# amathislab/BUCTD

Hardware: AMD Instinct MI355X
Metric: images/sec (train) BUCTD-CoAM-W48 384x288 (higher is better)
Workload: dtype f32 (3x3 convs: operands split exactly into 3 bf16 pieces, 6 bf16 MFMAs per product, fp32 accumulate - fp32-class); 1 GPU; BUCTD-CoAM-W48 (pose_hrnet_coam, ATT_MODULES [F,T,F,F], colored condition) 384x288 CrowdPose-14kpt full train step: fwd + JointsMSE + bwd + grad all-reduce + Adam + arg-max accuracy decode; global_batch=32, batch_per_gpu=32, input=N x 6 x 384 x 288 fp32, params=115581770, parallelism=dp1, hip_streams=4, conv_math=bf16x6, step_graph=False

## Files before the change

### buctd_amd/_C.py

```python
import ctypes as C
import os

import torch

_HERE = os.path.dirname(os.path.abspath(__file__))
LIB_PATH = os.path.join(_HERE, "lib", "libbuctd_hip.so")


class ConvDesc(C.Structure):
    _fields_ = [(n, C.c_int) for n in ("N", "H", "W", "Ci", "Co", "R", "S", "stride", "pad", "Ho", "Wo")]


class BasicBlockDesc(C.Structure):
    _fields_ = ([(n, C.c_int) for n in ("N", "H", "W", "C")] +
                [(n, C.c_void_p) for n in ("x", "w1_fwd", "w2_fwd", "w1_bwd", "w2_bwd", "gamma1", "beta1", "gamma2", "beta2",
                                           "running_mean1", "running_var1", "running_mean2", "running_var2")] +
                [(n, C.c_float) for n in ("eps1", "momentum1", "eps2", "momentum2")] +
                [(n, C.c_void_p) for n in ("z1", "z2", "y", "acc", "stat")])


class BasicBlockGrads(C.Structure):
    _fields_ = ([(n, C.c_void_p) for n in ("dy", "dz2", "dres", "dy1", "dz1", "dx", "dw1", "dw2", "dgamma1", "dbeta1",
                                           "dgamma2", "dbeta2")] +
                [(n, C.c_int) for n in ("acc_w1", "acc_w2", "acc_bn1", "acc_bn2")] +
# ... 9 lines not shown
class C3Conv(C.Structure):
    _fields_ = ([(n, C.c_int) for n in ("N", "H", "W", "Ci", "Co")] +
                [(n, C.c_void_p) for n in ("x", "wprep", "residual")] + [("relu", C.c_int)] +
                [(n, C.c_void_p) for n in ("y", "stats_acc")] + [("in_bn", C.POINTER(BnAccIn))] +
                [(n, C.c_void_p) for n in ("in_gamma", "in_beta")] + [("in_relu", C.c_int)] +
                [(n, C.c_void_p) for n in ("bn_z", "bn_y", "bn_mean", "bn_invstd", "bn_gamma", "bn_beta", "bn_acc")])


class C3ConvEval(C.Structure):
    _fields_ = ([(n, C.c_int) for n in ("N", "H", "W", "Ci", "Co")] +
                [(n, C.c_void_p) for n in ("x", "wprep", "scale", "shift", "residual")] + [("relu", C.c_int), ("y", C.c_void_p)])


class BnApplyItem(C.Structure):
    _fields_ = [("z", C.c_void_p), ("st", BnAccIn), ("gamma", C.c_void_p), ("beta", C.c_void_p), ("residual", C.c_void_p),
                ("relu", C.c_int), ("y", C.c_void_p), ("rows", C.c_long), ("C", C.c_int)]


class BnBwdItem(C.Structure):
    _fields_ = ([(n, C.c_void_p) for n in ("dy", "y", "z", "mean", "invstd", "gamma", "beta")] +
                [("relu", C.c_int), ("rows", C.c_long), ("C", C.c_int)] +
                [(n, C.c_void_p) for n in ("dz", "dres", "dgamma", "dbeta")] +
                [("accumulate", C.c_int), ("acc", C.c_void_p), ("acc_ready", C.c_int)])


class Wg3Conv(C.Structure):
    _fields_ = ([(n, C.c_int) for n in ("N", "H", "W", "Ci", "Co")] +
                [(n, C.c_void_p) for n in ("x", "dy", "dw")] + [("accumulate", C.c_int)] +
                [(n, C.c_void_p) for n in ("x_mean", "x_invstd", "x_gamma", "x_beta")] + [("x_relu", C.c_int)] +
                [("workspace", C.c_void_p), ("workspace_bytes", C.c_size_t)])


class MhaArgs(C.Structure):
    _fields_ = ([(n, C.c_int) for n in ("B", "T", "h", "dh")] +
                [(n, C.c_void_p) for n in ("q", "k", "v")] + [(n, C.c_int) for n in ("ldq", "ldk", "ldv")] +
                [("out", C.c_void_p), ("ldo", C.c_int), ("lse", C.c_void_p), ("scale", C.c_float), ("p_drop", C.c_float),
                 ("dout", C.c_void_p), ("lddo", C.c_int)] +
                [(n, C.c_void_p) for n in ("dq", "dk", "dv")] + [(n, C.c_int) for n in ("lddq", "lddk", "lddv")])


class RefineArgs(C.Structure):
    _fields_ = ([(n, C.c_void_p) for n in ("coords", "maxvals", "offset", "center", "scale", "box_score", "items",
                                           "cond_trunc", "cond_joints", "status", "hist_preds", "hist_score",
                                           "hist_box_score", "hist_keypoint_score", "hist_center", "hist_scale")] +
                [(n, C.c_int) for n in ("B", "K", "pass_", "passes", "heatmap_w", "heatmap_h", "crop_w", "crop_h")] +
                [(n, C.c_double) for n in ("margin", "aspect_ratio", "in_vis_thre", "scale_thre")])
# ... 135 lines not shown
    "buctd_joints_ohkm_mse_workspace": (_SZ, [_I, _I]),
    "buctd_joints_ohkm_mse": (_I, [_P, _P, _P, _I, _I, _I, _I, _P, _P, _F, _P, _SZ, _P]),
    "buctd_argmax_decode": (_I, [_P, _I, _I, _I, _P, _P, _P, _P]),
    "buctd_warp_affine_norm": (_I, [_P, _I, _I, _I, _P, _P, _P, _L, _P, _P]),
    "buctd_cond_render_into": (_I, [_P, _I, _P, _I, _I, _I, _I, _I, _I, _P, _L, _P, _SZ, _P]),
    "buctd_cond_geometry": (_I, [_P, _P, _P, _P, _I, _I, _P, _P, _P, _P]),
    "buctd_cond_mirror": (_I, [_P, _I, _P, _P, _I, _I, _I, _P, _P]),
    "buctd_mirror_rows": (_I, [_P, _L, _P, _L, _P, _I, _I, _I, _I, _I, _P]),
    "buctd_refine_step": (_I, [C.POINTER(RefineArgs), _P]),
    "buctd_sample_geometry": (_I, [C.POINTER(SampleGeomArgs), _P]),
    "buctd_synthesize_pose": (_I, [_P, _P, _P, _P, _P, _P, _I, _I, _I, C.c_ulonglong, _P, _P]),
    "buctd_mha_fwd_supported": (_I, [_I, _I]),
    "buctd_mha_fwd": (_I, [_I, _I, _I, _P, _P, _P, _I, _I, _F, _P, _P, _P]),
    "buctd_mha_fwd_bf16x6": (_I, [_I, _I, _I, _P, _P, _P, _I, _I, _F, _P, _P, _P]),
    "buctd_gconv_x6_supported": (_I, [_I] * 7),
    "buctd_gconv_x6_prep_bytes": (_SZ, [_I, _I, _I, _I]),
    "buctd_gconv_x6_prep": (_I, [_I, _I, _I, _P, _I, _P, _P]),
    "buctd_gconv_x6_prep_item_bytes": (_SZ, []),
    "buctd_gconv_x6_prep_item": (_I, [_I, _I, _I, _P, _I, _P, _P]),
    "buctd_gconv_x6_prep_batched": (_I, [_P, _I, _P]),
    "buctd_gconv_x6_stats_groups": (_I, [_I] * 6 + [_PI, _PI]),
    "buctd_gconv_x6_fwd": (_I, [_I] * 6 + [_P] * 6 + [_I, _P, _P, _P, _P]),
    "buctd_gconv_x6_dgrad": (_I, [_I] * 6 + [_P] * 4 + [_P]),
    "buctd_mha_fwd_bf16x6_workspace": (_SZ, [_I, _I, _I]),
    "buctd_mha_fwd_bf16x6_ws": (_I, [_I, _I, _I, _P, _P, _P, _I, _I, _F, _P, _P, _P, _SZ, _P]),
    "buctd_mha_train_supported": (_I, [_I, _I]),
    "buctd_mha_fwd_train": (_I, [_I, _I, _I, _P, _P, _P, _I, _I, _F, _F, _U64, _P, _P, _P]),
    "buctd_mha_bwd_workspace": (_SZ, [_I, _I]),
    "buctd_mha_bwd": (_I, [_I, _I, _I, _P, _P, _P, _I, _I, _P, _P, _P, _F, _F, _U64, _P, _P, _I, _P, _I, _P, _SZ, _P]),
    "buctd_mha_fwd_train_dseed": (_I, [_I, _I, _I, _P, _P, _P, _I, _I, _F, _F, _P, _P, _P, _P]),
    "buctd_mha_bwd_dseed": (_I, [_I, _I, _I, _P, _P, _P, _I, _I, _P, _P, _P, _F, _F, _P, _P, _P, _I, _P, _I, _P, _SZ, _P]),
    "buctd_mha_heads_fwd_supported": (_I, [_I, _I, _I]),
    "buctd_mha_heads_fwd": (_I, [C.POINTER(MhaArgs), _P]),
    "buctd_mha_heads_fwd_bf16x6": (_I, [C.POINTER(MhaArgs), _P]),
    "buctd_mha_heads_train_supported": (_I, [_I, _I, _I]),
    "buctd_mha_heads_fwd_train": (_I, [C.POINTER(MhaArgs), _U64, _P]),
    "buctd_mha_heads_bwd_workspace": (_SZ, [_I, _I, _I]),
    "buctd_mha_heads_bwd": (_I, [C.POINTER(MhaArgs), _U64, _P, _SZ, _P]),
    "buctd_mha_heads_fwd_train_dseed": (_I, [C.POINTER(MhaArgs), _P, _P]),
    "buctd_mha_heads_bwd_dseed": (_I, [C.POINTER(MhaArgs), _P, _P, _SZ, _P]),
    "buctd_nms_workspace": (_SZ, [_I]),
    "buctd_nms": (_I, [_P, _P, _P, _I, _I, _F, _P, _SZ, _P]),
    "buctd_cpu_nms": (_I, [_P, _I, _P, _F, _P, _P]),
    "buctd_argmax_decode_refined": (_I, [_P, _I, _I, _I, _P, _P, _P, _P, _P]),
    "buctd_argmax_decode_dark": (_I, [_P, _I, _I, _I, _P, _P, _P, _P, _P]),
    "buctd_gaussian_target": (_I, [_P, _P, _I, _I, _I, _I, _F, _F, _F, _P, _P, _P]),
# ... 61 lines not shown
```

### buctd_amd/csrc/conv_gather_x6.hip

```cpp
#include "c3_lean.h"
#include <string.h>

#define GC_MAXT 9
#define GC_TAB_OFF (56 * 1024)

struct GcClass {
  int ntaps, nhs, nsteps;
  int oy0, ox0;
  long wp_off;
  unsigned pdy, pdx;
};

struct GcArgs {
  C3Args e;
  const float* src;
  const unsigned char* wp;
  int SH, SWd, SC, ss, cpt;
  int ncls;
  GcClass cls[4];
};

template <int MF, int NF, int WM, int WN, int MODE>
__global__ __launch_bounds__(256, 2) void gconv_x6_kernel(GcArgs p) {
  constexpr int BM = WM * MF * 16, BN = WN * NF * 16, ROWB = 96, PST = 32, BROW = 192;
  constexpr int QA = BM / 64;
  static_assert(WM * WN == 4 && BM % 64 == 0, "four waves, BM a multiple of 64");
  extern __shared__ __attribute__((aligned(16))) unsigned char smem[];
  const int t = threadIdx.x, lane = t & 63, wave = t >> 6;
  const int i16 = lane & 15, g = lane >> 4;
  const int wave_m = wave % WM, wave_n = wave / WM;
  const int bx = blockIdx.x, by = blockIdx.y;
  const GcClass& c = p.cls[blockIdx.z];
  C3Args e = p.e;
  e.oy0 = c.oy0; e.ox0 = c.ox0;
  const int p0 = bx * BM, n0 = by * BN;

  constexpr bool PRIV = WN == 1;
  constexpr int RSTEP = PRIV ? 16 : 64;
  static_assert(!PRIV || MF * 16 / 16 == QA, "wave-private staging: MF passes of 16 rows == BM / 64");
  unsigned rowbase[QA];
  unsigned tapok[QA];
  const int arow = PRIV ? wave * (MF * 16) + (lane >> 2) : (t >> 2), c4 = t & 3;
  const __amdgpu_buffer_rsrc_t r_src = c3_rsrc(p.src, (unsigned)e.N * p.SH * p.SWd * p.SC * 4u);
#pragma unroll
  for (int q = 0; q < QA; ++q) {
    const int pp = p0 + arow + RSTEP * q;
    const int n = fast_div(pp, e.ib_mul, e.ib_sh);
    const int rem = pp - n * e.IB;
    const int yy = fast_div(rem, e.sw_mul, e.sw_sh), xx = rem - yy * e.SW;
    const bool real = (pp < e.P) & (n < e.N) & (yy >= 1) & (xx >= 1) & (xx <= e.W);
    const int sy0 = (yy - 1) * p.ss, sx0 = (xx - 1) * p.ss;
    rowbase[q] = (unsigned)(((n * p.SH + sy0) * p.SWd + sx0) * p.SC + c4 * 4) * 4u;
    unsigned ok = 0u;
    for (int tp = 0; tp < c.ntaps; ++tp) {
      const int sy = sy0 + (int)((c.pdy >> (2 * tp)) & 3u) - 1, sx = sx0 + (int)((c.pdx >> (2 * tp)) & 3u) - 1;
// ... 84 lines not shown
    if (2 * QA > MF) {
#pragma unroll
      for (int i = MF; i < 2 * QA; ++i) {
        const int h = i / QA, q = i % QA;
        split_store_pk<3, PST>(smem + (size_t)(1 - SET) * ABUF + ((size_t)h * BM + arow + RSTEP * q) * ROWB, c4 * 4,
                               areg[1 - SET][h][q]);
      }
    }
    if (!PRIV) __syncthreads();
  };

  load_a(0, areg[0]);
  load_b(0, bnx[0]);
  load_a(1, areg[1]);
  store_a(areg[0], 0);
  if (!PRIV) __syncthreads();
  for (int st = 0; st < c.nsteps; st += 2) {
    step(st, IC<0>{});
    if (st + 1 < c.nsteps) step(st + 1, IC<1>{});
  }
  __syncthreads();
  if constexpr (MODE < 0) c3_epilogue<MF, NF, WM, WN>(e, acc, smem, bx, by, p0, n0);
  else c3l_epilogue<MF, NF, WM, WN, MODE>(e, acc, smem, reinterpret_cast<float*>(smem + GC_TAB_OFF), p0, n0);
}

struct GcPrep {
  const float* w;
  unsigned char* out;
  int Co, Ci, R, S, dir;
  int ncls;
  int ntaps[4], nsteps[4];
  long off[4];
  int tr[4][GC_MAXT], ts[4][GC_MAXT];
  long items[4];
};

__device__ __forceinline__ void gc_prep_body(const GcPrep& p) {
  const int nrows = p.dir ? p.Ci : p.Co, kc = p.dir ? p.Co : p.Ci, cpt = kc / 16;
  const long total = p.items[p.ncls - 1];
  for (long idx = (long)blockIdx.x * 256 + threadIdx.x; idx < total; idx += (long)gridDim.x * 256) {
    int cl = 0;
    while (idx >= p.items[cl]) ++cl;
    const long li = idx - (cl ? p.items[cl - 1] : 0);
    const int ks = (int)(li & 31);
    const long sr = li >> 5;
    const int row = (int)(sr % nrows), st = (int)(sr / nrows);
// ... 329 lines not shown
static bool r1_ok(int kind, long rows, int cin, int cout) {
  if (kind != 1 || cin % 32 || (cout != 64 && cout != 128 && cout != 256)) return false;
  const size_t lds = (size_t)(cin / 32) * cout * R1_WROW + (size_t)8 * R1_STG;
  return lds <= 150 * 1024 && (size_t)8 * cout * 16 <= (size_t)(cin / 32) * cout * R1_WROW && rows >= 65536;
}

static int r1_run(long rows, int cin, int cout, const float* x, const void* wprep, const float* bias, const float* residual, float* out,
                  long long* stats_acc, hipStream_t st, const char* who) {
  R1Args a;
  a.x = x; a.wp = (const unsigned char*)wprep; a.bias = bias; a.res = residual; a.out = out; a.stats_acc = stats_acc;
  a.rows = rows; a.Ci = cin; a.Co = cout; a.nblocks = (int)((rows + 31) / 32);
  const size_t lds = (size_t)(cin / 32) * cout * R1_WROW + (size_t)8 * R1_STG;
  static unsigned char done[3][BUCTD_MAX_DEVICES] = {{0}};
  void (*fn)(R1Args) = cout == 64 ? conv1x1_rows_x6_kernel<4> : cout == 128 ? conv1x1_rows_x6_kernel<8> : conv1x1_rows_x6_kernel<16>;
  if (const int rc = buctd_raise_lds_limit(reinterpret_cast<const void*>(fn), 160 * 1024, done[cout == 64 ? 0 : cout == 128 ? 1 : 2], who))
    return rc;
  int grid = 256;
  if (grid * 8 > a.nblocks) grid = (a.nblocks + 7) / 8;
  hipLaunchKernelGGL(fn, dim3(grid), dim3(512), lds, st, a);
  BUCTD_CHECK_LAUNCH(who);
  return BUCTD_OK;
}

static int gc_run(int kind, int dir, int N, int H, int W, int Ci, int Co, const float* src, const void* wprep, const float* bias,
                  const float* scale, const float* shift, const float* residual, int relu, float* out, float* stats_partials,
                  int* stats_counts, void* stream, const char* who, long long* stats_acc = nullptr) {
  int Hg, Wg, SH, SWd, SC, nout;
  BUCTD_CHECK_ARG(src && wprep && out, "%s: null tensor pointer", who);
  BUCTD_CHECK_ARG(gc_geo(kind, dir, N, H, W, Ci, Co, &Hg, &Wg, &SH, &SWd, &SC, &nout),
                  "%s: unsupported shape kind %d N%d H%d W%d Ci%d Co%d", who, kind, N, H, W, Ci, Co);
  BUCTD_CHECK_ARG((scale == nullptr) == (shift == nullptr), "%s: scale and shift go together", who);
  BUCTD_CHECK_ARG((stats_partials == nullptr) == (stats_counts == nullptr), "%s: stats partials and counts go together", who);
  BUCTD_CHECK_ARG(!(dir && stats_partials), "%s: no statistics on the data gradient", who);
  if (!scale && !relu && !stats_partials && r1_ok(kind, (long)N * H * W, SC, nout))
    return r1_run((long)N * H * W, SC, nout, src, wprep, bias, residual, out, stats_acc, (hipStream_t)stream, who);
  GcPlan pl;
  gc_plan(nout, (long)N * (Hg + 1) * (Wg + 2) + Wg + 2, &pl);
  GcArgs a;
  C3Args& e = a.e;
  e.x = nullptr; e.wp = nullptr; e.out = out; e.bias = bias; e.scale = scale; e.shift = shift; e.res = residual;
  e.stats = stats_partials; e.counts = stats_counts;
  e.N = N; e.H = Hg; e.W = Wg; e.Ci = SC; e.Co = nout;
  e.SW = Wg + 2; e.IB = (Hg + 1) * (Wg + 2);
  e.P = (int)((long)N * e.IB + e.SW);
  e.relu = relu; e.na = 0;
  e.in_mean = e.in_invstd = e.in_gamma = e.in_beta = nullptr; e.in_relu = 0; e.col_major = 0;
  e.bs_z = e.bs_y = e.bs_mean = e.bs_invstd = e.bs_gamma = e.bs_beta = nullptr; e.bs_part = nullptr;
  e.stats_acc = stats_acc; e.bs_acc = nullptr;
  memset(&e.in_acc, 0, sizeof(e.in_acc));
  BUCTD_CHECK_ARG(!(dir && stats_acc), "%s: no statistics on the data gradient", who);
  magic_u32((unsigned)e.IB, &e.ib_mul, &e.ib_sh);
  magic_u32((unsigned)e.SW, &e.sw_mul, &e.sw_sh);
  const bool par = kind == 2 && dir;
  e.omap = par ? 1 : 0; e.oH = H; e.oW = W; e.ost = par ? 2 : 1; e.oy0 = e.ox0 = 0;
  a.src = src; a.wp = (const unsigned char*)wprep;
  a.SH = SH; a.SWd = SWd; a.SC = SC; a.ss = (kind == 2 && !dir) ? 2 : 1; a.cpt = SC / 16;
  a.ncls = gc_ncls(kind, dir);
  long off = 0;
  int tr[GC_MAXT], ts[GC_MAXT];
  for (int c = 0; c < 4; ++c) {
    GcClass& k = a.cls[c];
    k.ntaps = k.nhs = k.nsteps = 0; k.oy0 = k.ox0 = 0; k.wp_off = 0; k.pdy = k.pdx = 0u;
    if (c >= a.ncls) continue;
    int tdy[GC_MAXT], tdx[GC_MAXT];
    k.ntaps = gc_taps(kind, dir, c, tr, ts, tdy, tdx);
    k.pdy = k.pdx = 0u;
    for (int t = 0; t < k.ntaps; ++t) {
      k.pdy |= (unsigned)(tdy[t] + 1) << (2 * t);
      k.pdx |= (unsigned)(tdx[t] + 1) << (2 * t);
    }
    k.nhs = k.ntaps * a.cpt;
    k.nsteps = (k.nhs + 1) / 2;
    k.oy0 = par ? (c >> 1) : 0; k.ox0 = par ? (c & 1) : 0;
    k.wp_off = off;
    off += (long)gc_class_bytes(k.ntaps, SC, nout);
  }
  const int tiles = (e.P + pl.BM - 1) / pl.BM, ncol = nout / pl.BN;
  hipStream_t st = (hipStream_t)stream;
  int mode = -1;
  if (!bias && !scale && !relu && !stats_partials && !(stats_acc && residual) &&
      (long)N * H * W * (Ci > Co ? Ci : Co) * 4 < 2147483648L)
    mode = stats_acc ? C3M_STATS : residual ? C3M_RES : 0;
  if (pl.NF == 3 && pl.WM == 2) gc_launch<4, 3, 2, 2>(a, tiles, ncol, st, mode);
  else if (pl.NF == 4 && pl.WM == 2) gc_launch<4, 4, 2, 2>(a, tiles, ncol, st, mode);
  else if (pl.NF == 4) gc_launch<2, 4, 4, 1>(a, tiles, ncol, st, mode);
  else gc_launch<2, 3, 4, 1>(a, tiles, ncol, st, mode);
  BUCTD_CHECK_LAUNCH(who);
  return BUCTD_OK;
}

extern "C" int buctd_gconv_x6_fwd(int kind, int N, int H, int W, int Ci, int Co, const float* x, const void* wprep,
                                  const float* bias, const float* scale, const float* shift, const float* residual, int relu,
                                  float* y, float* stats_partials, int* stats_counts, void* stream) {
  return gc_run(kind, 0, N, H, W, Ci, Co, x, wprep, bias, scale, shift, residual, relu, y, stats_partials, stats_counts, stream,
                "buctd_gconv_x6_fwd");
}

extern "C" int buctd_gconv_x6_fwd_acc(int kind, int N, int H, int W, int Ci, int Co, const float* x, const void* wprep,
                                      const float* bias, float* y, void* stats_acc, void* stream) {
  BUCTD_CHECK_ARG(stats_acc, "buctd_gconv_x6_fwd_acc: null accumulator");
  return gc_run(kind, 0, N, H, W, Ci, Co, x, wprep, bias, nullptr, nullptr, nullptr, 0, y, nullptr, nullptr, stream,
                "buctd_gconv_x6_fwd_acc", (long long*)stats_acc);
}

extern "C" int buctd_gconv_x6_dgrad(int kind, int N, int H, int W, int Ci, int Co, const float* dy, const void* wprep,
                                    const float* residual, float* dx, void* stream) {
  return gc_run(kind, 1, N, H, W, Ci, Co, dy, wprep, nullptr, nullptr, nullptr, residual, 0, dx, nullptr, nullptr, stream,
                "buctd_gconv_x6_dgrad");
}
```

### buctd_amd/models/hrnet_common.py

```python
import logging
import os

import torch

from .. import nn
from .. import ops

BN_MOMENTUM = 0.1
logger = logging.getLogger(__name__)


def conv3x3(in_planes, out_planes, stride=1):
    return nn.Conv2d(in_planes, out_planes, kernel_size=3, stride=stride, padding=1, bias=False)


class BasicBlock(nn.Module):
    expansion = 1

    def __init__(self, inplanes, planes, stride=1, downsample=None):
        super().__init__()
        self.conv1 = conv3x3(inplanes, planes, stride)
        self.bn1 = nn.BatchNorm2d(planes, momentum=BN_MOMENTUM)
        self.relu = nn.ReLU(inplace=True)
        self.conv2 = conv3x3(planes, planes)
# ... 149 lines not shown
        outs = ops.fork_join([lambda p=p: ops.BasicBranchesFn.apply(chains[p[0]][0][0], [chains[i] for i in p], *[xs[i] for i in p])
                              for p in parts], [[xs[i] for i in p] for p in parts])
        ys = [None] * nb
        for p, o in zip(parts, outs):
            for i, y in zip(p, o):
                ys[i] = y
        return ys

    def _branches_grouped_eval(self, x):
        if self.training or torch.is_grad_enabled() or not all(type(br) is BlockChain and len(br) > 0 for br in self.branches):
            return None
        chains = []
        for br in self.branches:
            if not all(type(m) is BasicBlock and m.downsample is None and m.stride == 1 and m.conv1.bias is None
                       and m.conv2.bias is None and not m.bn1.training and not m.bn2.training
                       and m.bn1.running_mean is not None and m.bn2.running_mean is not None for m in br):
                return None
            chains.append([_block_params(m) for m in br])
        xs = [x[i] for i in range(self.num_branches)]
        if not ops.eval_branches_ok(xs, chains):
            return None
        return ops.basic_branches_eval(xs, chains)

    def forward(self, x):
        if self.num_branches == 1:
            return [self.branches[0](x[0])]
        xs = self._branches_grouped(x)
        if xs is None:
            xs = self._branches_grouped_eval(x)
        if xs is None:
            xs = ops.fork_join([lambda i=i: self.branches[i](x[i]) for i in range(self.num_branches)],
                               [x[i] for i in range(self.num_branches)])
        rows = list(enumerate(self.fuse_layers))
        fan = len(rows) > 1 and torch.is_grad_enabled() and any(t.requires_grad for t in xs)
        xr = [ops.FanOut.apply(xs[j], len(rows)) if fan and xs[j].is_cuda else [xs[j]] * len(rows)
              for j in range(self.num_branches)]

        def fuse_row(i, row):
            terms, shifts = [], []
            for j in range(self.num_branches):
                if j == i:
                    terms.append(xr[j][i])
                    shifts.append(0)
                elif j > i:
                    terms.append(row[j](xr[j][i]))
                    shifts.append(j - i)
                else:
                    terms.append(row[j](xr[j][i]))
                    shifts.append(0)
            return ops.FuseSum.apply(tuple(shifts), True, *terms)

        return ops.fork_join([lambda i=i, row=row: fuse_row(i, row) for i, row in rows], [xs for _ in rows], tag=1)


def make_transition_layer(pre, cur):
    layers = []
    for i in range(len(cur)):
        if i < len(pre):
            if cur[i] != pre[i]:
# ... 103 lines not shown
```

### buctd_amd/ops.py

```python
import ctypes as C
import math

import torch

from . import _C
from ._C import ConvDesc, MatmulDesc, check, lib, ptr, stream_ptr

_capture = {"on": False, "events": set(), "allow_seeds": False, "seed_table": None, "seed_draws": 0}
_SEED_TABLE_SLOTS = 1024


def capturing():
    return _capture["on"]


def _new_event(stream=None):
    ev = torch.cuda.Event()
    ev.record(stream) if stream is not None else ev.record()
    if _capture["on"]:
        _capture["events"].add(id(ev))
        _capture.setdefault("keep", []).append(ev)
    return ev


# ... 560 lines not shown

def _gconv_fwd(x, w, d, bias, scale, shift, residual, relu, stats):
    kind = _gconv_kind(d)
    wp = _gconv_prepared(w, kind, 0)
    y = torch.empty((d.N, d.Ho, d.Wo, d.Co), dtype=torch.float32, device=x.device)
    part = counts = info = None
    if stats == "acc" and scale is None and residual is None and not relu:
        acc = AccRef(d.Co, x.device)
        check(lib().buctd_gconv_x6_fwd_acc(kind, d.N, d.H, d.W, d.Ci, d.Co, ptr(x), ptr(wp), ptr(bias), ptr(y),
                                           C.c_void_p(acc.ptr), stream_ptr()), "gconv_x6_fwd_acc")
        return y, acc, ("acc",)
    if stats:
        def groups():
            ng, rpg = C.c_int(), C.c_int()
            check(lib().buctd_gconv_x6_stats_groups(kind, d.N, d.H, d.W, d.Ci, d.Co, C.byref(ng), C.byref(rpg)), "gconv groups")
            return ng.value, rpg.value
        ngv, rpgv = _memo(("gcgrp", kind, d.N, d.H, d.W, d.Ci, d.Co), groups)
        part = torch.empty((ngv, d.Co, 2), dtype=torch.float32, device=x.device)
        counts = torch.empty(ngv, dtype=torch.int32, device=x.device)
        info = (ngv, rpgv, counts)
    check(lib().buctd_gconv_x6_fwd(kind, d.N, d.H, d.W, d.Ci, d.Co, ptr(x), ptr(wp), ptr(bias), ptr(scale), ptr(shift),
                                   ptr(residual), int(bool(relu)), ptr(y), ptr(part), ptr(counts), stream_ptr()), "gconv_x6_fwd")
    return (y, part, info) if stats else y


_FUSED_BOTTLENECK = {"on": True}


def fused_bottleneck_on():
    return _FUSED_BOTTLENECK["on"]


def set_fused_bottleneck(on):
    old = _FUSED_BOTTLENECK["on"]
    _FUSED_BOTTLENECK["on"] = bool(on)
    return old


_FUSE_BN_IN = True
_MHA_X6 = True
_MHA_PRESPLIT = True
native_block_veto = {"fn": None}


def native_chain_ok(x_shape):
    return _conv_math["mode"] == "bf16x6" and native_block_veto["fn"] is None
# ... 737 lines not shown
    N, H, W, Cn = x_shape
    dx = torch.empty(tuple(x_shape), dtype=torch.float32, device=dy.device)
    check(lib().buctd_maxpool3x3s2_bwd(ptr(dy), ptr(idx), N, H, W, Cn, ptr(dx), stream_ptr()), "maxpool_bwd")
    return dx


def _contig(g):
    return g if g.is_contiguous() else g.contiguous()


def _count_batch(bn):
    bn.count_batch() if hasattr(bn, "count_batch") else bn.num_batches_tracked.add_(1)


class ConvBnAct(torch.autograd.Function):

    @staticmethod
    def forward(ctx, x, conv_w, conv_b, bn, residual, relu, stride, pad, training, transposed_shape):
        gamma, beta = bn.weight, bn.bias
        eps = bn.eps
        ctx.meta = (bn, conv_w, conv_b, relu, stride, pad, training, transposed_shape, tuple(x.shape))
        if training or bn.running_mean is None:
            momentum = 0.1 if bn.momentum is None else bn.momentum
            if transposed_shape is None:
                z, part, info = conv_fwd(x, conv_w, conv_b, stride, pad, stats="acc")
            else:
                z, part, info = conv_dgrad(x, conv_w, transposed_shape, stride, pad, bias=conv_b, stats="acc")
            Cn = z.shape[-1]
            rows = z.numel() // Cn
            track = bn.track_running_stats and training
            if info[0] == "acc":
                bnin = BnAccInput(part, rows, bn, training)
                y = bn_apply_acc(z, bnin, residual, relu)
                mean, invstd = bnin.mean, bnin.invstd
            else:
                mean, invstd = bn_finalize(part, info, rows, Cn, eps, momentum,
                                           bn.running_mean if track else None, bn.running_var if track else None)
                y = bn_apply(z, mean, invstd, gamma, beta, residual, relu)
            if track:
                _count_batch(bn)
            ctx.has_res = residual is not None
            ctx.save_for_backward(x, z, mean, invstd, y if (relu and ctx.has_res) else None)
            return y
        scale, shift = bn_fold_cached(bn, gamma, beta, eps)
        if transposed_shape is None:
            y = conv_fwd(x, conv_w, conv_b, stride, pad, scale=scale, shift=shift, residual=residual, relu=relu)
        else:
            z = conv_dgrad(x, conv_w, transposed_shape, stride, pad, bias=conv_b)
            Cn = z.shape[-1]
            zero = torch.zeros(Cn, dtype=torch.float32, device=z.device)
            y = bn_apply(z, zero, scale, torch.ones_like(zero), shift, residual, relu)
        ctx.save_for_backward()
        ctx.eval_mode = True
        return y

    @staticmethod
    def backward(ctx, dy):
        if getattr(ctx, "eval_mode", False):
            raise _C.BuctdHipError("backward through eval-mode BatchNorm is not on the BUCTD path")
        bn, conv_w, conv_b, relu, stride, pad, training, transposed_shape, x_shape = ctx.meta
        x, z, mean, invstd, y = ctx.saved_tensors
        dy = _contig(dy)
        dgamma, acc_g = grad_target(bn.weight)
        dbeta, acc_b = grad_target(bn.bias)
        assert acc_g == acc_b
        dz, dres = bn_bwd(dy, y, z, mean, invstd, bn.weight, relu, ctx.has_res and relu, dgamma, dbeta, acc_g, beta=bn.bias)
        if ctx.has_res and not relu:
            dres = dy
        dx = None
        if transposed_shape is None:
            if ctx.needs_input_grad[0]:
                dx = conv_dgrad(dz, conv_w, x_shape, stride, pad, residual=getattr(ctx, "dx_residual", None))
            dw, acc_w = grad_target(conv_w)
            conv_wgrad_async(x, dz, conv_w, stride, pad, dw, acc_w)
        else:
            if ctx.needs_input_grad[0]:
                dx = conv_fwd(dz, conv_w, None, stride, pad)
            dw, acc_w = grad_target(conv_w)
            conv_wgrad_async(dz, x, conv_w, stride, pad, dw, acc_w)
        if conv_b is not None:
            db, acc = grad_target(conv_b)
            colsum(dz, dz.shape[-1], db, acc)
        grad_done(bn.weight, bn.bias, conv_w, conv_b)
        return dx, None, None, None, dres, None, None, None, None, None


class _SubCtx:

    def __init__(self, needs_x=True):
        self.needs_input_grad = (needs_x,)
        self.saved_tensors = ()

    def save_for_backward(self, *tensors):
        self.saved_tensors = tensors
# ... 69 lines not shown
        for conv, bn, relu in groups:
            c = _SubCtx(need)
            s, p = conv._geom()
            outs.append(ConvBnAct.forward(c, x, conv.weight, conv.bias, bn, None, relu, s, p, True, None))
            subs.append(c)
        ctx.sub = subs
        _pack_subs(ctx, subs)
        return tuple(outs)

    @staticmethod
    def backward(ctx, *dys):
        subs = ctx.sub
        _unpack_subs(ctx, subs)
        dx = None
        for c, dy in zip(subs, dys):
            if dy is None:
                continue
            c.dx_residual = dx
            r = ConvBnAct.backward(c, dy)[0]
            dx = r if r is not None else dx
        for c in subs:
            c.saved_tensors = ()
        return dx, None, None


class BasicBlockFn(torch.autograd.Function):

    @staticmethod
    def forward(ctx, x, w1, bn1, w2, bn2):
        fuse = bn_in_fusable(tuple(x.shape), w2)
        veto = native_block_veto["fn"]
        if (fuse and bn_in_fusable(tuple(x.shape), w1) and bn1.track_running_stats == bn2.track_running_stats
                and not (veto is not None and veto(tuple(x.shape)))):
            ctx.native = True
            return _chain_forward(ctx, x, [(w1, bn1, w2, bn2)])
        ctx.native = False
        z1, part, info = conv_fwd(x, w1, None, 1, 1, stats="acc")
        Cn = z1.shape[-1]
        rows = z1.numel() // Cn
        y1 = None
        if info[0] == "acc":
            bnin1 = BnAccInput(part, rows, bn1, True, relu=True)
            if fuse:
                z2, part2, info2 = conv_fwd(z1, w2, None, 1, 1, stats="acc", in_bn=bnin1)
            else:
                y1 = bn_apply_acc(z1, bnin1, None, True)
# ... 800 lines not shown
```

### include/buctd_hip.h

```cpp
#ifndef BUCTD_HIP_H
#define BUCTD_HIP_H
#include <stddef.h>
#include <stdint.h>

#ifdef __cplusplus
extern "C" {
#endif

int buctd_version(void);
const char* buctd_last_error(void);

typedef struct {
  int N, H, W, Ci;
  int Co, R, S;
  int stride, pad;
  int Ho, Wo;
} buctd_conv_desc;

int buctd_conv2d_fwd_thin(const buctd_conv_desc* d);
int buctd_conv2d_fwd(const buctd_conv_desc* d, const float* x, const float* w, const float* bias,
                     const float* scale, const float* shift, const float* residual, int relu, float* y,
                     float* stats_partials, void* stream);
int buctd_conv2d_dgrad(const buctd_conv_desc* d, const float* dy, const float* w, const float* bias, float* dx,
                       float* stats_partials, void* stream);
// ... 242 lines not shown
                             float* offset, void* stream);
int buctd_gaussian_target(const float* joints, const float* vis, int B, int K, int Hh, int Wh, float stride_x,
                          float stride_y, float sigma, float* target, float* weight, void* stream);
size_t buctd_cond_render_workspace(int B, int Cc, int H, int W);
int buctd_cond_render(const float* joints, int js, const float* colors, int B, int K, int Cc, int H, int W,
                      int truncate, float* cond, void* workspace, size_t workspace_bytes, void* stream);
int buctd_flipback_avg(const float* a, const float* b, const int32_t* perm, int N, int K, int H, int W, int shift,
                       float* out, void* stream);

int buctd_gconv_x6_supported(int kind, int N, int H, int W, int Ci, int Co, int dir);
size_t buctd_gconv_x6_prep_bytes(int kind, int Ci, int Co, int dir);
int buctd_gconv_x6_prep(int kind, int Ci, int Co, const float* w, int dir, void* wprep, void* stream);
size_t buctd_gconv_x6_prep_item_bytes(void);
int buctd_gconv_x6_prep_item(int kind, int Ci, int Co, const float* w, int dir, void* wprep, void* item_host);
int buctd_gconv_x6_prep_batched(const void* items_device, int n, void* stream);
int buctd_gconv_x6_stats_groups(int kind, int N, int H, int W, int Ci, int Co, int* ngroups, int* rows_per_group);
int buctd_gconv_x6_fwd(int kind, int N, int H, int W, int Ci, int Co, const float* x, const void* wprep, const float* bias,
                       const float* scale, const float* shift, const float* residual, int relu, float* y,
                       float* stats_partials, int* stats_counts, void* stream);
int buctd_gconv_x6_fwd_acc(int kind, int N, int H, int W, int Ci, int Co, const float* x, const void* wprep, const float* bias,
                           float* y, void* stats_acc, void* stream);
int buctd_gconv_x6_dgrad(int kind, int N, int H, int W, int Ci, int Co, const float* dy, const void* wprep,
                         const float* residual, float* dx, void* stream);
int buctd_gconv_wgrad_x6_supported(int kind, int N, int H, int W, int Ci, int Co);
size_t buctd_gconv_wgrad_x6_workspace(int kind, int N, int H, int W, int Ci, int Co);
int buctd_gconv_wgrad_x6(int kind, int N, int H, int W, int Ci, int Co, const float* x, const float* dy, float* dw,
                         int accumulate, void* workspace, size_t workspace_bytes, void* stream);

typedef struct {
  int N, H, W, C;
  const float* x;
  const void *w1_fwd, *w2_fwd;
  const void *w1_bwd, *w2_bwd;
  const float *gamma1, *beta1, *gamma2, *beta2;
  float *running_mean1, *running_var1, *running_mean2, *running_var2;
  float eps1, momentum1, eps2, momentum2;
  float *z1, *z2, *y;
  void* acc;
  float* stat;
} buctd_basic_block;
typedef struct {
  const float* dy;
  float *dz2, *dres, *dy1, *dz1;
  float* dx;
  float *dw1, *dw2, *dgamma1, *dbeta1, *dgamma2, *dbeta2;
  int acc_w1, acc_w2, acc_bn1, acc_bn2;
// ... 184 lines not shown
```

Measured before the change: 509.4 images/s.

## Batch HRNet fuse-layer gather convs into grouped launches per level

Adds a grouped gather-conv kernel that packs up to seven independent conv problems into one launch, decoding member, tile and class from a flat workgroup index. Members are sorted by step count. The HRNet fuse stage gains a level-by-level path that runs all cross-branch ConvBN forwards, BN applies, BN backwards and deferred data gradients as grouped calls. The aim is fewer small kernel launches and better GPU fill for the many tiny downsample/upsample convs. The cost is a larger kernel-argument payload and more complex autograd bookkeeping.

```diff
diff --git a/buctd_amd/_C.py b/buctd_amd/_C.py
--- a/buctd_amd/_C.py
+++ b/buctd_amd/_C.py
@@ -55,6 +55,11 @@
                 [("relu", C.c_int), ("rows", C.c_long), ("C", C.c_int)] +
                 [(n, C.c_void_p) for n in ("dz", "dres", "dgamma", "dbeta")] +
                 [("accumulate", C.c_int), ("acc", C.c_void_p), ("acc_ready", C.c_int)])
+
+
+class GconvItem(C.Structure):
+    _fields_ = ([(n, C.c_int) for n in ("kind", "N", "H", "W", "Ci", "Co")] +
+                [(n, C.c_void_p) for n in ("src", "wprep", "bias", "residual", "out", "stats_acc")])
 
 
 class Wg3Conv(C.Structure):
@@ -236,6 +241,10 @@
     "buctd_gconv_x6_stats_groups": (_I, [_I] * 6 + [_PI, _PI]),
     "buctd_gconv_x6_fwd": (_I, [_I] * 6 + [_P] * 6 + [_I, _P, _P, _P, _P]),
     "buctd_gconv_x6_dgrad": (_I, [_I] * 6 + [_P] * 4 + [_P]),
+    "buctd_gconv_x6_fwd_acc_group": (_I, [_I, C.POINTER(GconvItem), _P]),
+    "buctd_gconv_x6_dgrad_group": (_I, [_I, C.POINTER(GconvItem), _P]),
+    "buctd_gconv_x6_group_workgroups": (_I, [_I, C.POINTER(GconvItem)]),
+    "buctd_gconv_x6_group_launches": (_I, [_I, C.POINTER(GconvItem)]),
     "buctd_mha_fwd_bf16x6_workspace": (_SZ, [_I, _I, _I]),
     "buctd_mha_fwd_bf16x6_ws": (_I, [_I, _I, _I, _P, _P, _P, _I, _I, _F, _P, _P, _P, _SZ, _P]),
     "buctd_mha_train_supported": (_I, [_I, _I]),
diff --git a/buctd_amd/csrc/conv_gather_x6.hip b/buctd_amd/csrc/conv_gather_x6.hip
--- a/buctd_amd/csrc/conv_gather_x6.hip
+++ b/buctd_amd/csrc/conv_gather_x6.hip
@@ -21,16 +21,14 @@
 };
 
 template <int MF, int NF, int WM, int WN, int MODE>
-__global__ __launch_bounds__(256, 2) void gconv_x6_kernel(GcArgs p) {
+__device__ __forceinline__ void gc_tile(const GcArgs& p, unsigned char* smem, int bx, int by, int bz) {
   constexpr int BM = WM * MF * 16, BN = WN * NF * 16, ROWB = 96, PST = 32, BROW = 192;
   constexpr int QA = BM / 64;
   static_assert(WM * WN == 4 && BM % 64 == 0, "four waves, BM a multiple of 64");
-  extern __shared__ __attribute__((aligned(16))) unsigned char smem[];
   const int t = threadIdx.x, lane = t & 63, wave = t >> 6;
   const int i16 = lane & 15, g = lane >> 4;
   const int wave_m = wave % WM, wave_n = wave / WM;
-  const int bx = blockIdx.x, by = blockIdx.y;
-  const GcClass& c = p.cls[blockIdx.z];
+  const GcClass& c = p.cls[bz];
   C3Args e = p.e;
   e.oy0 = c.oy0; e.ox0 = c.ox0;
   const int p0 = bx * BM, n0 = by * BN;
@@ -161,6 +159,35 @@
   __syncthreads();
   if constexpr (MODE < 0) c3_epilogue<MF, NF, WM, WN>(e, acc, smem, bx, by, p0, n0);
   else c3l_epilogue<MF, NF, WM, WN, MODE>(e, acc, smem, reinterpret_cast<float*>(smem + GC_TAB_OFF), p0, n0);
+}
+
+template <int MF, int NF, int WM, int WN, int MODE>
+__global__ __launch_bounds__(256, 2) void gconv_x6_kernel(GcArgs p) {
+  extern __shared__ __attribute__((aligned(16))) unsigned char smem[];
+  gc_tile<MF, NF, WM, WN, MODE>(p, smem, blockIdx.x, blockIdx.y, blockIdx.z);
+}
+
+#define GCG_MAX 7
+#define GCG_REQ_MAX 16
+struct GcGroup {
+  GcArgs m[GCG_MAX];
+  int n;
+  unsigned first[GCG_MAX + 1];
+  int tiles[GCG_MAX], ncol[GCG_MAX];
+};
+static_assert(sizeof(GcGroup) <= 4096, "GcGroup travels in the kernel-argument segment");
+
+template <int MF, int NF, int WM, int WN, int MODE>
+__global__ __launch_bounds__(256, 2) void gconv_x6_group_kernel(GcGroup g_) {
+  extern __shared__ __attribute__((aligned(16))) unsigned char smem[];
+  const GcGroup& g = *(const GcGroup*)__builtin_amdgcn_kernarg_segment_ptr();
+  int k = 0;
+  while (k + 1 < g.n && blockIdx.x >= g.first[k + 1]) ++k;
+  const unsigned lid = blockIdx.x - g.first[k];
+  const unsigned tiles = (unsigned)g.tiles[k], per = tiles * (unsigned)g.ncol[k];
+  const unsigned bz = lid / per, rem = lid - bz * per;
+  const unsigned by = rem / tiles, bx = rem - by * tiles;
+  gc_tile<MF, NF, WM, WN, MODE>(g.m[k], smem, (int)bx, (int)by, (int)bz);
 }
 
 struct GcPrep {
@@ -536,9 +563,16 @@
   return BUCTD_OK;
 }
 
-static int gc_run(int kind, int dir, int N, int H, int W, int Ci, int Co, const float* src, const void* wprep, const float* bias,
-                  const float* scale, const float* shift, const float* residual, int relu, float* out, float* stats_partials,
-                  int* stats_counts, void* stream, const char* who, long long* stats_acc = nullptr) {
+struct GcLaunch {
+  GcArgs a;
+  GcPlan pl;
+  int tiles, ncol, mode;
+  bool rows;
+};
+
+static int gc_fill(GcLaunch* L, int kind, int dir, int N, int H, int W, int Ci, int Co, const float* src, const void* wprep,
+                   const float* bias, const float* scale, const float* shift, const float* residual, int relu, float* out,
+                   float* stats_partials, int* stats_counts, const char* who, long long* stats_acc) {
   int Hg, Wg, SH, SWd, SC, nout;
   BUCTD_CHECK_ARG(src && wprep && out, "%s: null tensor pointer", who);
   BUCTD_CHECK_ARG(gc_geo(kind, dir, N, H, W, Ci, Co, &Hg, &Wg, &SH, &SWd, &SC, &nout),
@@ -546,11 +580,12 @@
   BUCTD_CHECK_ARG((scale == nullptr) == (shift == nullptr), "%s: scale and shift go together", who);
   BUCTD_CHECK_ARG((stats_partials == nullptr) == (stats_counts == nullptr), "%s: stats partials and counts go together", who);
   BUCTD_CHECK_ARG(!(dir && stats_partials), "%s: no statistics on the data gradient", who);
-  if (!scale && !relu && !stats_partials && r1_ok(kind, (long)N * H * W, SC, nout))
-    return r1_run((long)N * H * W, SC, nout, src, wprep, bias, residual, out, stats_acc, (hipStream_t)stream, who);
-  GcPlan pl;
+  BUCTD_CHECK_ARG(!(dir && stats_acc), "%s: no statistics on the data gradient", who);
+  L->rows = !scale && !relu && !stats_partials && r1_ok(kind, (long)N * H * W, SC, nout);
+  if (L->rows) return BUCTD_OK;
+  GcPlan& pl = L->pl;
   gc_plan(nout, (long)N * (Hg + 1) * (Wg + 2) + Wg + 2, &pl);
-  GcArgs a;
+  GcArgs& a = L->a;
   C3Args& e = a.e;
   e.x = nullptr; e.wp = nullptr; e.out = out; e.bias = bias; e.scale = scale; e.shift = shift; e.res = residual;
   e.stats = stats_partials; e.counts = stats_counts;
@@ -562,7 +597,6 @@
   e.bs_z = e.bs_y = e.bs_mean = e.bs_invstd = e.bs_gamma = e.bs_beta = nullptr; e.bs_part = nullptr;
   e.stats_acc = stats_acc; e.bs_acc = nullptr;
   memset(&e.in_acc, 0, sizeof(e.in_acc));
-  BUCTD_CHECK_ARG(!(dir && stats_acc), "%s: no statistics on the data gradient", who);
   magic_u32((unsigned)e.IB, &e.ib_mul, &e.ib_sh);
   magic_u32((unsigned)e.SW, &e.sw_mul, &e.sw_sh);
   const bool par = kind == 2 && dir;
@@ -589,12 +623,27 @@
     k.wp_off = off;
     off += (long)gc_class_bytes(k.ntaps, SC, nout);
   }
-  const int tiles = (e.P + pl.BM - 1) / pl.BM, ncol = nout / pl.BN;
-  hipStream_t st = (hipStream_t)stream;
-  int mode = -1;
+  L->tiles = (e.P + pl.BM - 1) / pl.BM;
+  L->ncol = nout / pl.BN;
+  L->mode = -1;
   if (!bias && !scale && !relu && !stats_partials && !(stats_acc && residual) &&
       (long)N * H * W * (Ci > Co ? Ci : Co) * 4 < 2147483648L)
-    mode = stats_acc ? C3M_STATS : residual ? C3M_RES : 0;
+    L->mode = stats_acc ? C3M_STATS : residual ? C3M_RES : 0;
+  return BUCTD_OK;
+}
+
+static int gc_run(int kind, int dir, int N, int H, int W, int Ci, int Co, const float* src, const void* wprep, const float* bias,
+                  const float* scale, const float* shift, const float* residual, int relu, float* out, float* stats_partials,
+                  int* stats_counts, void* stream, const char* who, long long* stats_acc = nullptr) {
+  GcLaunch L;
+  if (const int rc = gc_fill(&L, kind, dir, N, H, W, Ci, Co, src, wprep, bias, scale, shift, residual, relu, out, stats_partials,
+                             stats_counts, who, stats_acc))
+    return rc;
+  hipStream_t st = (hipStream_t)stream;
+  if (L.rows) return r1_run((long)N * H * W, dir ? Co : Ci, dir ? Ci : Co, src, wprep, bias, residual, out, stats_acc, st, who);
+  const GcArgs& a = L.a;
+  const GcPlan& pl = L.pl;
+  const int tiles = L.tiles, ncol = L.ncol, mode = L.mode;
   if (pl.NF == 3 && pl.WM == 2) gc_launch<4, 3, 2, 2>(a, tiles, ncol, st, mode);
   else if (pl.NF == 4 && pl.WM == 2) gc_launch<4, 4, 2, 2>(a, tiles, ncol, st, mode);
   else if (pl.NF == 4) gc_launch<2, 4, 4, 1>(a, tiles, ncol, st, mode);
@@ -622,3 +671,98 @@
   return gc_run(kind, 1, N, H, W, Ci, Co, dy, wprep, nullptr, nullptr, nullptr, residual, 0, dx, nullptr, nullptr, stream,
                 "buctd_gconv_x6_dgrad");
 }
+
+static int gc_plan_index(const GcPlan& pl) { return (pl.NF == 3 && pl.WM == 2) ? 0 : (pl.NF == 4 && pl.WM == 2) ? 1 : pl.NF == 4 ? 2 : 3; }
+
+template <int MF, int NF, int WM, int WN>
+static void gcg_launch(const GcGroup& g, hipStream_t st, int mode) {
+  constexpr int BN = WN * NF * 16;
+  const dim3 grid(g.first[g.n]);
+  const size_t lds = GC_TAB_OFF + 4 * BN * 4;
+  if (mode == C3M_STATS) hipLaunchKernelGGL((gconv_x6_group_kernel<MF, NF, WM, WN, C3M_STATS>), grid, dim3(256), lds, st, g);
+  else if (mode == C3M_RES) hipLaunchKernelGGL((gconv_x6_group_kernel<MF, NF, WM, WN, C3M_RES>), grid, dim3(256), lds, st, g);
+  else hipLaunchKernelGGL((gconv_x6_group_kernel<MF, NF, WM, WN, 0>), grid, dim3(256), lds, st, g);
+}
+
+static int gcg_run(int n, const buctd_gconv_item* items, int dir, bool launch, void* stream, const char* who, long* nwg, int* nlaunch) {
+  BUCTD_CHECK_ARG(items && n > 0 && n <= GCG_REQ_MAX, "%s: 1..%d members", who, GCG_REQ_MAX);
+  hipStream_t st = (hipStream_t)stream;
+  GcLaunch L[GCG_REQ_MAX];
+  unsigned char done[GCG_REQ_MAX] = {0};
+  int rc = BUCTD_OK;
+  for (int i = 0; i < n && !rc; ++i) {
+    const buctd_gconv_item& it = items[i];
+    if (dir && (it.bias || it.stats_acc)) { buctd_set_error("%s: member %d: no bias or statistics on the data gradient", who, i); rc = BUCTD_EINVAL; break; }
+    if (!dir && (!it.stats_acc || it.residual)) { buctd_set_error("%s: member %d: the forward needs an accumulator and takes no residual", who, i); rc = BUCTD_EINVAL; break; }
+    rc = gc_fill(&L[i], it.kind, dir, it.N, it.H, it.W, it.Ci, it.Co, it.src, it.wprep, it.bias, nullptr, nullptr, it.residual, 0, it.out,
+                 nullptr, nullptr, who, (long long*)it.stats_acc);
+  }
+  long wg = 0;
+  int nl = 0;
+  for (int i = 0; i < n && !rc; ++i) {
+    if (done[i]) continue;
+    const buctd_gconv_item& it = items[i];
+    if (L[i].rows || L[i].mode < 0) {
+      done[i] = 1;
+      if (!L[i].rows) { wg += (long)L[i].tiles * L[i].ncol * L[i].a.ncls; ++nl; }
+      if (launch)
+        rc = gc_run(it.kind, dir, it.N, it.H, it.W, it.Ci, it.Co, it.src, it.wprep, it.bias, nullptr, nullptr, it.residual, 0, it.out, nullptr,
+                    nullptr, stream, who, (long long*)it.stats_acc);
+      continue;
+    }
+    const int pi = gc_plan_index(L[i].pl), mode = L[i].mode;
+    int idx[GCG_MAX], cnt = 0;
+    for (int j = i; j < n && cnt < GCG_MAX; ++j)
+      if (!done[j] && !L[j].rows && L[j].mode == mode && gc_plan_index(L[j].pl) == pi) { idx[cnt++] = j; done[j] = 1; }
+    for (int a = 1; a < cnt; ++a)
+      for (int b = a; b > 0; --b) {
+        int sa = 0, sb = 0;
+        for (int c = 0; c < 4; ++c) { sa = L[idx[b - 1]].a.cls[c].nsteps > sa ? L[idx[b - 1]].a.cls[c].nsteps : sa; sb = L[idx[b]].a.cls[c].nsteps > sb ? L[idx[b]].a.cls[c].nsteps : sb; }
+        if (sb <= sa) break;
+        const int tmp = idx[b]; idx[b] = idx[b - 1]; idx[b - 1] = tmp;
+      }
+    GcGroup g;
+    memset(&g, 0, sizeof(g));
+    g.n = cnt;
+    g.first[0] = 0;
+    for (int k = 0; k < cnt; ++k) {
+      const GcLaunch& m = L[idx[k]];
+      g.m[k] = m.a;
+      g.tiles[k] = m.tiles; g.ncol[k] = m.ncol;
+      g.first[k + 1] = g.first[k] + (unsigned)(m.tiles * m.ncol * m.a.ncls);
+    }
+    for (int k = cnt; k < GCG_MAX; ++k) g.first[k + 1] = g.first[cnt];
+    wg += g.first[cnt];
+    ++nl;
+    if (launch) {
+      if (pi == 0) gcg_launch<4, 3, 2, 2>(g, st, mode);
+      else if (pi == 1) gcg_launch<4, 4, 2, 2>(g, st, mode);
+      else if (pi == 2) gcg_launch<2, 4, 4, 1>(g, st, mode);
+      else gcg_launch<2, 3, 4, 1>(g, st, mode);
+      if (hipGetLastError() != hipSuccess) { buctd_set_error("%s: kernel launch failed", who); rc = BUCTD_EINVAL; }
+    }
+  }
+  if (nwg) *nwg = wg;
+  if (nlaunch) *nlaunch = nl;
+  return rc;
+}
+
+extern "C" int buctd_gconv_x6_fwd_acc_group(int n, const buctd_gconv_item* items, void* stream) {
+  return gcg_run(n, items, 0, true, stream, "buctd_gconv_x6_fwd_acc_group", nullptr, nullptr);
+}
+
+extern "C" int buctd_gconv_x6_dgrad_group(int n, const buctd_gconv_item* items, void* stream) {
+  return gcg_run(n, items, 1, true, stream, "buctd_gconv_x6_dgrad_group", nullptr, nullptr);
+}
+
+extern "C" int buctd_gconv_x6_group_workgroups(int n, const buctd_gconv_item* items) {
+  long wg = 0;
+  const int dir = (items && n > 0 && items[0].stats_acc) ? 0 : 1;
+  return gcg_run(n, items, dir, false, nullptr, "buctd_gconv_x6_group_workgroups", &wg, nullptr) ? -1 : (int)wg;
+}
+
+extern "C" int buctd_gconv_x6_group_launches(int n, const buctd_gconv_item* items) {
+  int nl = 0;
+  const int dir = (items && n > 0 && items[0].stats_acc) ? 0 : 1;
+  return gcg_run(n, items, dir, false, nullptr, "buctd_gconv_x6_group_launches", nullptr, &nl) ? -1 : nl;
+}
diff --git a/buctd_amd/models/hrnet_common.py b/buctd_amd/models/hrnet_common.py
--- a/buctd_amd/models/hrnet_common.py
+++ b/buctd_amd/models/hrnet_common.py
@@ -195,6 +195,38 @@
             return None
         return ops.basic_branches_eval(xs, chains)
 
+    def _fuse_levels(self, xr, rows):
+        nb = self.num_branches
+        if not (self.training and torch.is_grad_enabled() and ops.fuse_level_ok() and all(t[0].is_cuda for t in xr)):
+            return None
+        levels = {}
+        for i, row in rows:
+            for j in range(nb):
+                if j == i:
+                    continue
+                steps = [row[j]] if j > i else list(row[j])
+                if not all(type(m) is nn.ConvBN and m[1].training for m in steps):
+                    return None
+                for k, m in enumerate(steps):
+                    levels.setdefault(k, []).append((i, j, m))
+        if not any(ops.fuse_level_groupable(tuple(xr[j][i].shape), m[0]) for i, j, m in levels.get(0, [])):
+            return None
+        cur = {}
+        for k in sorted(levels):
+            mem = levels[k]
+            for _, _, m in mem:
+                nn._as_channels_last_(m[0].weight)
+            ins = [xr[j][i] if k == 0 else cur[(i, j)] for i, j, _ in mem]
+            outs = ops.FuseLevelFn.apply(mem[0][2][0].weight, [(m[0], m[1], m._relu) for _, _, m in mem], *ins)
+            for (i, j, _), y in zip(mem, outs):
+                cur[(i, j)] = y
+        ys = []
+        for i, _ in rows:
+            terms = [xr[j][i] if j == i else cur[(i, j)] for j in range(nb)]
+            shifts = [j - i if j > i else 0 for j in range(nb)]
+            ys.append(ops.FuseSum.apply(tuple(shifts), True, *terms))
+        return ys
+
     def forward(self, x):
         if self.num_branches == 1:
             return [self.branches[0](x[0])]
@@ -208,6 +240,10 @@
         fan = len(rows) > 1 and torch.is_grad_enabled() and any(t.requires_grad for t in xs)
         xr = [ops.FanOut.apply(xs[j], len(rows)) if fan and xs[j].is_cuda else [xs[j]] * len(rows)
               for j in range(self.num_branches)]
+
+        ys = self._fuse_levels(xr, rows)
+        if ys is not None:
+            return ys
 
         def fuse_row(i, row):
             terms, shifts = [], []
diff --git a/buctd_amd/ops.py b/buctd_amd/ops.py
--- a/buctd_amd/ops.py
+++ b/buctd_amd/ops.py
@@ -606,6 +606,45 @@
     check(lib().buctd_gconv_x6_fwd(kind, d.N, d.H, d.W, d.Ci, d.Co, ptr(x), ptr(wp), ptr(bias), ptr(scale), ptr(shift),
                                    ptr(residual), int(bool(relu)), ptr(y), ptr(part), ptr(counts), stream_ptr()), "gconv_x6_fwd")
     return (y, part, info) if stats else y
+
+
+gconv_group_calls = {"fwd": 0, "dgrad": 0}
+
+
+def _gconv_items(members, direction):
+    arr = (_C.GconvItem * len(members))()
+    for it, (src, w, d, residual, out, acc) in zip(arr, members):
+        kind = _gconv_kind(d)
+        it.kind, it.N, it.H, it.W, it.Ci, it.Co = kind, d.N, d.H, d.W, d.Ci, d.Co
+        it.src, it.wprep = ptr(src), ptr(_gconv_prepared(w, kind, direction))
+        it.bias, it.residual, it.out = None, ptr(residual), ptr(out)
+        it.stats_acc = acc.ptr if acc is not None else None
+    return arr
+
+
+def gconv_fwd_acc_group(members):
+    full = []
+    for x, w, d in members:
+        _f32(x, "conv input")
+        weight_rsc(w)
+        full.append((x, w, d, None, torch.empty((d.N, d.Ho, d.Wo, d.Co), dtype=torch.float32, device=x.device),
+                     AccRef(d.Co, x.device)))
+    check(lib().buctd_gconv_x6_fwd_acc_group(len(full), _gconv_items(full, 0), stream_ptr()), "gconv_x6_fwd_acc_group")
+    gconv_group_calls["fwd"] += 1
+    return [(m[4], m[5], ("acc",)) for m in full]
+
+
+def gconv_dgrad_group(members):
+    full = []
+    for dy, w, d, residual in members:
+        _f32(dy, "conv dgrad input")
+        weight_rsc(w)
+        if tuple(dy.shape) != (d.N, d.Ho, d.Wo, d.Co):
+            raise _C.BuctdHipError(f"conv_dgrad: dy shape {tuple(dy.shape)} != {(d.N, d.Ho, d.Wo, d.Co)}")
+        full.append((dy, w, d, residual, torch.empty((d.N, d.H, d.W, d.Ci), dtype=torch.float32, device=dy.device), None))
+    check(lib().buctd_gconv_x6_dgrad_group(len(full), _gconv_items(full, 1), stream_ptr()), "gconv_x6_dgrad_group")
+    gconv_group_calls["dgrad"] += 1
+    return [m[4] for m in full]
 
 
 _FUSED_BOTTLENECK = {"on": True}
@@ -1389,7 +1428,10 @@
         ctx.meta = (bn, conv_w, conv_b, relu, stride, pad, training, transposed_shape, tuple(x.shape))
         if training or bn.running_mean is None:
             momentum = 0.1 if bn.momentum is None else bn.momentum
-            if transposed_shape is None:
+            pre = getattr(ctx, "pre_conv", None)
+            if pre is not None:
+                z, part, info = pre
+            elif transposed_shape is None:
                 z, part, info = conv_fwd(x, conv_w, conv_b, stride, pad, stats="acc")
             else:
                 z, part, info = conv_dgrad(x, conv_w, transposed_shape, stride, pad, bias=conv_b, stats="acc")
@@ -1436,7 +1478,9 @@
             dres = dy
         dx = None
         if transposed_shape is None:
-            if ctx.needs_input_grad[0]:
+            if ctx.needs_input_grad[0] and getattr(ctx, "defer_dgrad", False):
+                ctx.dz = dz
+            elif ctx.needs_input_grad[0]:
                 dx = conv_dgrad(dz, conv_w, x_shape, stride, pad, residual=getattr(ctx, "dx_residual", None))
             dw, acc_w = grad_target(conv_w)
             conv_wgrad_async(x, dz, conv_w, stride, pad, dw, acc_w)
@@ -1552,6 +1596,135 @@
         for c in subs:
             c.saved_tensors = ()
         return dx, None, None
+
+
+def fuse_level_ok():
+    return _conv_math["mode"] == "bf16x6" and native_block_veto["fn"] is None
+
+
+def fuse_level_groupable(x_shape, conv):
+    if conv.bias is not None:
+        return False
+    s, p = conv._geom()
+    d = conv_desc(x_shape, _wshape(conv.weight), s, p)
+    return _gconv_ok(d, 0) or _gconv_ok(d, 1)
+
+
+class FuseLevelFn(torch.autograd.Function):
+
+    @staticmethod
+    def forward(ctx, w0, members, *xs):
+        geo, grouped = [], []
+        for k, ((conv, bn, relu), x) in enumerate(zip(members, xs)):
+            s, p = conv._geom()
+            d = conv_desc(x.shape, _wshape(conv.weight), s, p)
+            geo.append((s, p, d))
+            if conv.bias is None and _gconv_ok(d, 0):
+                grouped.append(k)
+        pre = dict(zip(grouped, gconv_fwd_acc_group([(xs[k], members[k][0].weight, geo[k][2]) for k in grouped]))) if grouped else {}
+        for k, ((conv, bn, relu), x) in enumerate(zip(members, xs)):
+            if k not in pre:
+                pre[k] = conv_fwd(x, conv.weight, conv.bias, geo[k][0], geo[k][1], stats="acc")
+        bng = [k for k in range(len(members)) if pre[k][2][0] == "acc" and members[k][0].bias is None and bn_acc_ok(pre[k][0].shape[-1])]
+        bnins = {k: BnAccInput(pre[k][1], pre[k][0].numel() // pre[k][0].shape[-1], members[k][1], True) for k in bng}
+        ys = dict(zip(bng, _bn_apply_acc_group([(pre[k][0], bnins[k], members[k][2]) for k in bng])))
+        subs, outs = [], []
+        for k, ((conv, bn, relu), x) in enumerate(zip(members, xs)):
+            c = _SubCtx(ctx.needs_input_grad[2 + k])
+            s, p, d = geo[k]
+            c.bn_group = k in ys
+            if c.bn_group:
+                c.meta = (bn, conv.weight, None, relu, s, p, True, None, tuple(x.shape))
+                c.has_res = False
+                if bn.track_running_stats:
+                    _count_batch(bn)
+                c.save_for_backward(x, pre[k][0], bnins[k].mean, bnins[k].invstd, None)
+                outs.append(ys[k])
+            else:
+                c.pre_conv = pre[k]
+                outs.append(ConvBnAct.forward(c, x, conv.weight, conv.bias, bn, None, relu, s, p, True, None))
+                c.pre_conv = None
+            c.defer_dgrad = conv.bias is None and _gconv_ok(d, 1)
+            c.desc = d
+            subs.append(c)
+        ctx.sub = subs
+        _pack_subs(ctx, subs)
+        return tuple(outs)
+
+    @staticmethod
+    def backward(ctx, *dys):
+        subs = ctx.sub
+        _unpack_subs(ctx, subs)
+        dxs = [None] * len(subs)
+        live = [k for k, dy in enumerate(dys) if dy is not None]
+        bng = [k for k in live if subs[k].bn_group]
+        items = []
+        for k in bng:
+            c = subs[k]
+            bn, relu = c.meta[0], c.meta[3]
+            x, z, mean, invstd, _ = c.saved_tensors
+            dgamma, acc_g = grad_target(bn.weight)
+            dbeta, acc_b = grad_target(bn.bias)
+            assert acc_g == acc_b
+            items.append((_contig(dys[k]), z, mean, invstd, bn.weight, bn.bias if relu else None, relu, dgamma, dbeta, acc_g))
+        for k, dz in zip(bng, _bn_bwd_acc_group(items)):
+            subs[k].dz = dz
+        for k in live:
+            c = subs[k]
+            if not c.bn_group:
+                c.dz = None
+                dxs[k] = ConvBnAct.backward(c, dys[k])[0]
+                continue
+            bn, conv_w, _, relu, s, p, _, _, x_shape = c.meta
+            x, dz = c.saved_tensors[0], c.dz
+            if c.needs_input_grad[0] and not c.defer_dgrad:
+                dxs[k] = conv_dgrad(dz, conv_w, x_shape, s, p)
+            dw, acc_w = grad_target(conv_w)
+            conv_wgrad_async(x, dz, conv_w, s, p, dw, acc_w)
+            grad_done(bn.weight, bn.bias, conv_w)
+            if not (c.needs_input_grad[0] and c.defer_dgrad):
+                c.dz = None
+        late = [k for k in live if getattr(subs[k], "dz", None) is not None]
+        if late:
+            for k, dx in zip(late, gconv_dgrad_group([(subs[k].dz, subs[k].meta[1], subs[k].desc, None) for k in late])):
+                dxs[k] = dx
+        for c in subs:
+            c.saved_tensors = ()
+            c.dz = None
+        return (None, None, *dxs)
+
+
+def _bn_apply_acc_group(members):
+    ys = []
+    for g0 in range(0, len(members), 4):
+        chunk = members[g0:g0 + 4]
+        arr = (_C.BnApplyItem * len(chunk))()
+        for it, (z, bnin, relu) in zip(arr, chunk):
+            Cn = z.shape[-1]
+            y = torch.empty_like(z)
+            it.z, it.st, it.gamma, it.beta, it.residual = ptr(z), bnin.struct(), ptr(bnin.gamma), ptr(bnin.beta), None
+            it.relu, it.y, it.rows, it.C = int(bool(relu)), ptr(y), z.numel() // Cn, Cn
+            ys.append(y)
+        check(lib().buctd_bn_apply_acc_group(len(chunk), arr, stream_ptr()), "bn_apply_acc_group")
+    return ys
+
+
+def _bn_bwd_acc_group(members):
+    dzs = []
+    for g0 in range(0, len(members), 4):
+        chunk = members[g0:g0 + 4]
+        arr = (_C.BnBwdItem * len(chunk))()
+        for it, (dy, z, mean, invstd, gamma, beta, relu, dgamma, dbeta, accumulate) in zip(arr, chunk):
+            Cn = z.shape[-1]
+            dz = torch.empty_like(z)
+            acc = AccRef(Cn, z.device)
+            it.dy, it.y, it.z, it.mean, it.invstd, it.gamma, it.beta = ptr(dy), None, ptr(z), ptr(mean), ptr(invstd), ptr(gamma), ptr(beta)
+            it.relu, it.rows, it.C = int(bool(relu)), z.numel() // Cn, Cn
+            it.dz, it.dres, it.dgamma, it.dbeta, it.accumulate = ptr(dz), None, ptr(dgamma), ptr(dbeta), int(accumulate)
+            it.acc, it.acc_ready = acc.ptr, 0
+            dzs.append(dz)
+        check(lib().buctd_bn_bwd_acc_group(len(chunk), arr, stream_ptr()), "bn_bwd_acc_group")
+    return dzs
 
 
 class BasicBlockFn(torch.autograd.Function):
diff --git a/include/buctd_hip.h b/include/buctd_hip.h
--- a/include/buctd_hip.h
+++ b/include/buctd_hip.h
@@ -288,6 +288,19 @@
                            float* y, void* stats_acc, void* stream);
 int buctd_gconv_x6_dgrad(int kind, int N, int H, int W, int Ci, int Co, const float* dy, const void* wprep,
                          const float* residual, float* dx, void* stream);
+typedef struct {
+  int kind, N, H, W, Ci, Co;
+  const float* src;
+  const void* wprep;
+  const float* bias;
+  const float* residual;
+  float* out;
+  void* stats_acc;
+} buctd_gconv_item;
+int buctd_gconv_x6_fwd_acc_group(int n, const buctd_gconv_item* items, void* stream);
+int buctd_gconv_x6_dgrad_group(int n, const buctd_gconv_item* items, void* stream);
+int buctd_gconv_x6_group_workgroups(int n, const buctd_gconv_item* items);
+int buctd_gconv_x6_group_launches(int n, const buctd_gconv_item* items);
 int buctd_gconv_wgrad_x6_supported(int kind, int N, int H, int W, int Ci, int Co);
 size_t buctd_gconv_wgrad_x6_workspace(int kind, int N, int H, int W, int Ci, int Co);
 int buctd_gconv_wgrad_x6(int kind, int N, int H, int W, int Ci, int Co, const float* x, const float* dy, float* dw,
```

Measured after the change: 510.4 images/s, median of 6. No clear change (+0.2%).
